# jackyko1991/vnet-tensorflow

Measured on AMD Instinct MI355X. Metric: training patches/sec (128^3x1ch fp32), higher is better.
Workload: dtype f32

## Files before the change

### include/vnet_hip.h

```cpp
#ifndef VNET_HIP_H
#define VNET_HIP_H
#include <stddef.h>
#include <stdint.h>

#ifdef __cplusplus
extern "C" {
#endif

#define VNET_OK            0
#define VNET_E_BADARG     -1
#define VNET_E_UNSUPPORTED -2
#define VNET_E_WORKSPACE  -3

#define VNET_ACT_NONE  0
#define VNET_ACT_RELU  1
#define VNET_ACT_PRELU 2
#define VNET_ACT_LRELU 3

#define VNET_PACK_FWD  0
#define VNET_PACK_BWD  1
#define VNET_PACK_UP   2

#define VNET_PACK_FWD_BF16 3
#define VNET_PACK_BWD_BF16 4
// ... 9 lines not shown
#define VNET_LOSS_SORENSEN 0
#define VNET_LOSS_JACCARD  1
#define VNET_LOSS_XENT     2
#define VNET_LOSS_WEIGHTED 16
#define VNET_LOSS_MIXED    32

const char* vnet_version(void);

double vnet_set_option(const char* name, double value);
double vnet_get_option(const char* name);

size_t vnet_packed_weight_floats(int mode, int taps, int I, int O);
int vnet_pack_weights(int mode, const float* w, float* wp, int taps, int I, int O, void* stream);
int vnet_packed_dims(int mode, int taps, int I, int O, int* CQ, int* NP);
int vnet_pack_weights_batched(const void* descs_dev, int n, void* stream);

size_t vnet_conv_ws_bytes(int ks, int kx, int stride, int up, int Cin, int Cout, int B, int Do, int Ho, int Wo);
int vnet_conv_fwd(int ks, int kx, int stride, int up, const float* x0, int C0, const float* x1, int C1, const float* wp,
    const float* bias, float* y0, int Cy0, float* y1, int Cy1, int B, int Di, int Hi, int Wi, int Do, int Ho, int Wo, void* ws,
    size_t ws_bytes, void* stream);

int vnet_conv_fwd_acc(int ks, int kx, int stride, int up, const float* x0, int C0, const float* x1, int C1, const float* wp,
    const float* bias, float* y0, int Cy0, float* y1, int Cy1, int B, int Di, int Hi, int Wi, int Do, int Ho, int Wo, void* ws,
    size_t ws_bytes, void* stream);

int vnet_conv_stats_rows(int ks, int kx, int stride, int up, int Cin, int Cy0, int Cy1, int B, int Do, int Ho, int Wo);
int vnet_conv_stats_from_reduce(int ks, int kx, int stride, int Cin, int Cout, int B, int Do, int Ho, int Wo);
int vnet_conv_fwd_stats(int ks, int kx, int stride, const float* x0, int C0, const float* x1, int C1, const float* wp,
    const float* bias, float* y, int Cout, int B, int Di, int Hi, int Wi, int Do, int Ho, int Wo, const float* res, float* stats,
    void* ws, size_t ws_bytes, void* stream);

int vnet_conv_x3_ok(int C0, int C1, int Cy0, int Cy1, int B, int D, int H, int W);
int vnet_conv_x3_stats_rows(int Cin, int Cout, int B, int D, int H, int W);
size_t vnet_conv_x3_ws_bytes(int Cin, int Cout, int B, int D, int H, int W);
int vnet_conv_fwd_x3(const float* x0, int C0, const float* x1, int C1, const void* wp, const float* bias, float* y0, int Cy0,
    float* y1, int Cy1, int B, int D, int H, int W, const float* acc, const float* res, float* stats, void* ws, size_t ws_bytes,
    void* stream);

int vnet_wgrad_x3_ok(int C0, int C1, int Cout, int B, int D, int H, int W);
size_t vnet_wgrad_x3_ws_bytes(int Cin, int Cout, int B, int D, int H, int W);
int vnet_conv_wgrad_x3(const float* x0, int C0, const float* x1, int C1, const float* dy, int Cout, float* dw, int B, int D, int H,
    int W, void* ws, size_t ws_bytes, void* stream);

size_t vnet_wgrad_bf16_ws_bytes(int Cin, int Cout, int B, int D, int H, int W);

int vnet_wgrad_defer(int on, void* stream);
int vnet_wgrad_pending(void* stream);
int vnet_wgrad_flush(void* stream);

size_t vnet_wgrad_ws_bytes(int ks, int kx, int stride, int Cin, int Cout, int B, int Do, int Ho, int Wo);
int vnet_conv_wgrad(int ks, int kx, int stride, const float* x0, int C0, const float* x1, int C1, const float* dy, int Cout,
    float* dw, int B, int Di, int Hi, int Wi, int Do, int Ho, int Wo, void* ws, size_t ws_bytes, void* stream);

int vnet_tile_im2col_x(const float* img, float* xv, int B, int D, int H, int W, void* stream);
int vnet_input_conv_fold(const float* w, const float* gamma, const float* beta, const float* mean, const float* invstd, float* wv,
    int C, int O, void* stream);
int vnet_input_conv_grads(const float* G, const float* w, const float* gamma, const float* beta, const float* mean,
    const float* invstd, float* dw, float* dgamma, float* dbeta, int C, int O, int accumulate, void* stream);

int vnet_input_conv_direct_ok(int O, int B, int D, int H, int W);
int vnet_input_conv_direct_stats_rows(int B, int D, int H, int W);
int vnet_input_conv_fold_border(const float* wv, int O, float* wbc , float* cbc , void* stream);
int vnet_input_conv_direct_fwd(const float* img, const float* wv, const float* wbc, const float* cbc, const float* bias, const float* res,
    float* y, float* stats, int O, int B, int D, int H, int W, void* stream);
int vnet_input_wgrad_direct_slabs(int B, int D, int H, int W);
int vnet_input_wgrad_direct(const float* img, const float* dy, float* G, int O, int B, int D, int H, int W, void* ws, size_t ws_bytes,
// ... 150 lines not shown
```

### vnet_tensorflow_amd/_lib.py

```python
import ctypes
import os
import subprocess

_HERE = os.path.dirname(os.path.abspath(__file__))
LIB_PATH = os.environ.get("VNET_HIP_LIB") or os.path.join(_HERE, "libvnet_hip.so")
CSRC = os.path.join(_HERE, "csrc")

_vp, _i, _i64, _f, _sz, _u64, _d = (ctypes.c_void_p, ctypes.c_int, ctypes.c_int64, ctypes.c_float,
                                    ctypes.c_size_t, ctypes.c_uint64, ctypes.c_double)

SIGNATURES = {
    "vnet_version": (ctypes.c_char_p, []),
    "vnet_set_option": (_d, [ctypes.c_char_p, _d]),
    "vnet_get_option": (_d, [ctypes.c_char_p]),
    "vnet_packed_weight_floats": (_sz, [_i, _i, _i, _i]),
    "vnet_pack_weights": (_i, [_i, _vp, _vp, _i, _i, _i, _vp]),
    "vnet_packed_dims": (_i, [_i, _i, _i, _i, ctypes.POINTER(ctypes.c_int), ctypes.POINTER(ctypes.c_int)]),
    "vnet_pack_weights_batched": (_i, [_vp, _i, _vp]),
    "vnet_conv_x3_ok": (_i, [_i] * 8),
    "vnet_conv_x3_stats_rows": (_i, [_i] * 6),
    "vnet_conv_x3_ws_bytes": (_sz, [_i] * 6),
    "vnet_conv_fwd_x3": (_i, [_vp, _i, _vp, _i, _vp, _vp, _vp, _i, _vp, _i, _i, _i, _i, _i, _vp, _vp, _vp, _vp, _sz, _vp]),
    "vnet_wgrad_x3_ok": (_i, [_i] * 7),
    "vnet_wgrad_x3_ws_bytes": (_sz, [_i] * 6),
    "vnet_conv_wgrad_x3": (_i, [_vp, _i, _vp, _i, _vp, _i, _vp, _i, _i, _i, _i, _vp, _sz, _vp]),
    "vnet_conv_ws_bytes": (_sz, [_i, _i, _i, _i, _i, _i, _i, _i, _i, _i]),
    "vnet_conv_fwd": (_i, [_i, _i, _i, _i, _vp, _i, _vp, _i, _vp, _vp, _vp, _i, _vp, _i,
                           _i, _i, _i, _i, _i, _i, _i, _vp, _sz, _vp]),
    "vnet_conv_fwd_acc": (_i, [_i, _i, _i, _i, _vp, _i, _vp, _i, _vp, _vp, _vp, _i, _vp, _i,
                               _i, _i, _i, _i, _i, _i, _i, _vp, _sz, _vp]),
    "vnet_conv_stats_rows": (_i, [_i] * 11),
    "vnet_conv_stats_from_reduce": (_i, [_i] * 9),
    "vnet_conv_fwd_stats": (_i, [_i, _i, _i, _vp, _i, _vp, _i, _vp, _vp, _vp, _i,
                                 _i, _i, _i, _i, _i, _i, _i, _vp, _vp, _vp, _sz, _vp]),
    "vnet_bn_finalize_partial": (_i, [_vp, _i, _i, _d, _f, _f, _vp, _vp, _vp, _vp, _vp]),
    "vnet_colsum_b16_ws_bytes": (_sz, [_i]),
    "vnet_colsum_b16": (_i, [_vp, _vp, _i64, _i, _vp, _sz, _vp]),
    "vnet_conv_b16_ws_bytes": (_sz, [_i] * 8),
    "vnet_conv_b16_stats_rows": (_i, [_i] * 8),
    "vnet_wgrad_bf16_ws_bytes": (_sz, [_i, _i, _i, _i, _i, _i]),
    "vnet_wgrad_defer": (_i, [_i, _vp]),
    "vnet_wgrad_pending": (_i, [_vp]),
    "vnet_wgrad_flush": (_i, [_vp]),
    "vnet_wgrad_ws_bytes": (_sz, [_i, _i, _i, _i, _i, _i, _i, _i, _i]),
    "vnet_conv_wgrad": (_i, [_i, _i, _i, _vp, _i, _vp, _i, _vp, _i, _vp,
                             _i, _i, _i, _i, _i, _i, _i, _vp, _sz, _vp]),
    "vnet_tile_im2col_x": (_i, [_vp, _vp, _i, _i, _i, _i, _vp]),
    "vnet_input_conv_fold": (_i, [_vp, _vp, _vp, _vp, _vp, _vp, _i, _i, _vp]),
    "vnet_input_conv_grads": (_i, [_vp, _vp, _vp, _vp, _vp, _vp, _vp, _vp, _vp, _i, _i, _i, _vp]),
    "vnet_input_conv_direct_ok": (_i, [_i, _i, _i, _i, _i]),
    "vnet_input_conv_direct_stats_rows": (_i, [_i, _i, _i, _i]),
    "vnet_input_conv_fold_border": (_i, [_vp, _i, _vp, _vp, _vp]),
    "vnet_input_conv_direct_fwd": (_i, [_vp, _vp, _vp, _vp, _vp, _vp, _vp, _vp, _i, _i, _i, _i, _i, _vp]),
# ... 140 lines not shown
```

### vnet_tensorflow_amd/csrc/conv_kernels.h

```cpp
#pragma once
#include "common.h"
#include <mutex>
#include <unordered_map>
#include <type_traits>
#include <vector>

namespace {

struct ConvArgs {
    const float* x0; const float* x1; int C0, C1, Cin;
    const float4* wp; const float* bias;
    float* y0; float* y1; int Cy0, Cy1, Cout;
    int B, Di, Hi, Wi, Do, Ho, Wo;
    int CQ;
    int CoutP;
    int nchunks, cps;
    int nbz, nby, nbx;
    int pad, padx;
    int vec_in, vec_out;
    float* part; size_t part_stride;
    int upO;
    int nz;
    int accum;
    const float* accsrc;
    float* stats; const float* res;
    int in4;
};

#ifdef VNET_STAMPS
static __device__ long long* g_stamps = nullptr;
#define VNET_STAMP_DECL long long ts[12]; bool stamp_on = false
#define VNET_STAMP_STEP(step) stamp_on = blockIdx.x == 88 && (step) >= 4 && (step) < 8
#define VNET_STAMP(k) do { if (stamp_on) ts[k] = __builtin_readcyclecounter(); } while (0)
#define VNET_STAMP_FLUSH(step, wave, lane, n) do { if (stamp_on && (lane) == 0 && g_stamps) { \
        for (int q_ = 0; q_ < (n); ++q_) g_stamps[(((step) - 4) * 8 + (wave)) * 12 + q_] = ts[q_]; } } while (0)
#else
#define VNET_STAMP_DECL
#define VNET_STAMP_STEP(step)
#define VNET_STAMP(k) do {} while (0)
#define VNET_STAMP_FLUSH(step, wave, lane, n) do {} while (0)
#endif

__device__ __forceinline__ float row16_sum(float v) {
    v += __builtin_bit_cast(float, __builtin_amdgcn_update_dpp(0, __builtin_bit_cast(int, v), 0xB1, 0xf, 0xf, true));
    v += __builtin_bit_cast(float, __builtin_amdgcn_update_dpp(0, __builtin_bit_cast(int, v), 0x4E, 0xf, 0xf, true));
    v += __builtin_bit_cast(float, __builtin_amdgcn_update_dpp(0, __builtin_bit_cast(int, v), 0x141, 0xf, 0xf, true));
    v += __builtin_bit_cast(float, __builtin_amdgcn_update_dpp(0, __builtin_bit_cast(int, v), 0x140, 0xf, 0xf, true));
    return v;
}
__device__ __forceinline__ float half32_sum(float v) {
    v = row16_sum(v);
    return v + __shfl_xor(v, 16, 64);
}

template <int WAVES_, int CW>
__device__ __forceinline__ void stats_row_write(const float* red, float* __restrict__ stats, size_t row, int co0, int Cout, int tid) {
    if (tid < 2 * CW) {
        float t = 0.f;
#pragma unroll
        for (int w = 0; w < WAVES_; ++w) t += red[w * 2 * CW + tid];
        const int a2 = tid / CW, c = co0 + (tid - a2 * CW);
        if (c < Cout) stats[row * 2 * Cout + (size_t)a2 * Cout + c] = t;
    }
}

__device__ __forceinline__ float bf_lo(uint32_t w) { return __uint_as_float(w << 16); }
__device__ __forceinline__ float bf_hi(uint32_t w) { return __uint_as_float(w & 0xffff0000u); }
template <bool STATS>
__device__ __forceinline__ void epilogue4_b16(const ConvArgs& a, size_t ov, int co, float (&e)[4], float* s1, float* s2) {
    unsigned short* y = (co < a.Cy0) ? reinterpret_cast<unsigned short*>(a.y0) + ov * a.Cy0 + co
                                     : reinterpret_cast<unsigned short*>(a.y1) + ov * a.Cy1 + (co - a.Cy0);
    if (a.accum) {
        const unsigned short* src = a.accsrc ? reinterpret_cast<const unsigned short*>(a.accsrc) + ov * a.Cy0 + co : y;
        const uint2 o = *reinterpret_cast<const uint2*>(src);
        e[0] += bf_lo(o.x); e[1] += bf_hi(o.x); e[2] += bf_lo(o.y); e[3] += bf_hi(o.y);
    }
    const uint2 pk = make_uint2(pk_bf16(e[0], e[1]), pk_bf16(e[2], e[3]));
    if constexpr (STATS) {
        float v[4] = {bf_lo(pk.x), bf_hi(pk.x), bf_lo(pk.y), bf_hi(pk.y)};
        if (a.res) {
            const uint2 r = *reinterpret_cast<const uint2*>(reinterpret_cast<const unsigned short*>(a.res) + ov * a.Cout + co);
            v[0] += bf_lo(r.x); v[1] += bf_hi(r.x); v[2] += bf_lo(r.y); v[3] += bf_hi(r.y);
        }
#pragma unroll
        for (int k = 0; k < 4; ++k) { s1[k] += v[k]; s2[k] += v[k] * v[k]; }
    }
    *reinterpret_cast<uint2*>(y) = pk;
}

template <bool STATS, int N>
__device__ __forceinline__ void epilogue_b16_batch(const ConvArgs& a, const size_t (&ov)[N], const int (&co)[N], const bool (&ok)[N],
                                                   float (&e)[N][4]) {
    unsigned short* y[N];
    uint2 old[N], rr[N];
#pragma unroll
// ... 520 lines not shown
        if (sg == 0 && idx < total) {
            float out[W];
#pragma unroll
            for (int j = 0; j < W; ++j) out[j] = sh[0][o * W + j] + sh[1][o * W + j] + sh[2][o * W + j] + sh[3][o * W + j];
            if (VEC) *reinterpret_cast<float4*>(dw + idx * 4) = make_float4(out[0], out[W > 1 ? 1 : 0], out[W > 2 ? 2 : 0], out[W > 3 ? 3 : 0]);
            else dw[idx] = out[0];
        }
    }
}

template <bool VEC>
__global__ void __launch_bounds__(256) wgrad_reduce_kernel(const float* __restrict__ part, int nsplit, int T3, int CinP, int CoutP,
                                                           int Cin, int Cout, float* __restrict__ dw) {
    wgrad_reduce_body<VEC>(part, nsplit, T3, CinP, CoutP, Cin, Cout, dw, blockIdx.x, gridDim.x);
}

}
namespace vnet_detail {
struct ReduceJob { const float* part; float* dw; int nsplit, T3, CinP, CoutP, Cin, Cout, vec; unsigned blk0; };
constexpr int REDUCE_BATCH = 32;
struct ReduceBatch { ReduceJob job[REDUCE_BATCH]; int n; };
struct DeferQueue { bool on = false; std::vector<ReduceJob> pending; };
struct DeferState { std::mutex mu; std::unordered_map<hipStream_t, DeferQueue> q; };
__attribute__((visibility("hidden"))) DeferState& defer_state();
struct Tuning {
    int wgrad_zs;
    int wgrad_rr;
    int conv_in4;
    double group_rounds;
    int group_debug;
    int bf16_deep;
    int bf16_deep_target;
    int bf16_c16pp;
    int x3_nb2;
    int f32_small;
};
__attribute__((visibility("hidden"))) Tuning& tuning();
}
namespace {
using vnet_detail::ReduceJob; using vnet_detail::ReduceBatch; using vnet_detail::REDUCE_BATCH;
using vnet_detail::DeferState; using vnet_detail::DeferQueue; using vnet_detail::defer_state; using vnet_detail::tuning;

__global__ void __launch_bounds__(256) wgrad_reduce_batched_kernel(ReduceBatch b) {
    int j = 0;
#pragma unroll 1
    for (int k = 1; k < b.n; ++k) if (blockIdx.x >= b.job[k].blk0) j = k;
    const ReduceJob& q = b.job[j];
    const unsigned nblk = (j + 1 < b.n ? b.job[j + 1].blk0 : gridDim.x) - q.blk0;
    if (q.vec) wgrad_reduce_body<true>(q.part, q.nsplit, q.T3, q.CinP, q.CoutP, q.Cin, q.Cout, q.dw, blockIdx.x - q.blk0, nblk);
    else wgrad_reduce_body<false>(q.part, q.nsplit, q.T3, q.CinP, q.CoutP, q.Cin, q.Cout, q.dw, blockIdx.x - q.blk0, nblk);
}


int launch_wgrad_reduce(const float* part, int nsplit, int T3, int CinP, int CoutP, int Cin, int Cout, float* dw, hipStream_t st) {
    const bool vec = (Cout % 4 == 0) && (CoutP % 4 == 0) && ((reinterpret_cast<uintptr_t>(dw) | reinterpret_cast<uintptr_t>(part)) & 15) == 0;
    {
        DeferState& ds = defer_state();
        std::lock_guard<std::mutex> lk(ds.mu);
        auto it = ds.q.find(st);
        if (it != ds.q.end() && it->second.on) {
            it->second.pending.push_back(ReduceJob{part, dw, nsplit, T3, CinP, CoutP, Cin, Cout, vec ? 1 : 0, 0u});
            return 0;
        }
    }
    const size_t total = (size_t)T3 * Cin * Cout / (vec ? 4 : 1);
    const int blocks = (int)min((size_t)4096, (total + 63) / 64);
// ... 1638 lines not shown
```

### vnet_tensorflow_amd/csrc/conv_mfma.hip

```cpp
#include "conv_kernels.h"
#include <string.h>

namespace vnet_detail {
DeferState& defer_state() { static DeferState s; return s; }
static Tuning tuning_from_env() {
    auto geti = [](const char* n, int d) { const char* e = getenv(n); return e ? atoi(e) : d; };
    Tuning t{};
    t.wgrad_zs = geti("VNET_WGRAD_ZS", 2); t.wgrad_rr = geti("VNET_WGRAD_RR", 1); t.conv_in4 = geti("VNET_CONV_IN4", 1);
    const char* g = getenv("VNET_WGRAD_GROUP_ROUNDS");
    t.group_rounds = g ? atof(g) : 2.0;
    t.group_debug = getenv("VNET_WGRAD_GROUP_DEBUG") ? 1 : 0;
    t.bf16_deep = geti("VNET_BF16_DEEP", 1); t.bf16_deep_target = geti("VNET_BF16_DEEP_TARGET", 256);
    t.f32_small = geti("VNET_F32_SMALL", 2); t.x3_nb2 = geti("VNET_X3_NB2", 1); t.bf16_c16pp = geti("VNET_BF16_C16PP", 1);
    return t;
}
Tuning& tuning() { static Tuning t = tuning_from_env(); return t; }
}

namespace {
double* option_slot(const char* name, int** ip) {
    vnet_detail::Tuning& t = vnet_detail::tuning();
    *ip = nullptr;
    if (!name) return nullptr;
    if (!strcmp(name, "WGRAD_ZS")) *ip = &t.wgrad_zs;
    else if (!strcmp(name, "WGRAD_RR")) *ip = &t.wgrad_rr;
    else if (!strcmp(name, "CONV_IN4")) *ip = &t.conv_in4;
    else if (!strcmp(name, "WGRAD_GROUP_DEBUG")) *ip = &t.group_debug;
    else if (!strcmp(name, "BF16_DEEP")) *ip = &t.bf16_deep;
    else if (!strcmp(name, "BF16_DEEP_TARGET")) *ip = &t.bf16_deep_target;
    else if (!strcmp(name, "F32_SMALL")) *ip = &t.f32_small;
    else if (!strcmp(name, "X3_NB2")) *ip = &t.x3_nb2;
    else if (!strcmp(name, "BF16_C16PP")) *ip = &t.bf16_c16pp;
    else if (!strcmp(name, "WGRAD_GROUP_ROUNDS")) return &t.group_rounds;
    return nullptr;
}
}

extern "C" {

double vnet_set_option(const char* name, double value) {
    int* ip; double* dp = option_slot(name, &ip);
    if (ip) { const double prev = *ip; *ip = (int)value; return prev; }
    if (dp) { const double prev = *dp; *dp = value; return prev; }
    return __builtin_nan("");
}
double vnet_get_option(const char* name) {
    int* ip; double* dp = option_slot(name, &ip);
    return ip ? (double)*ip : (dp ? *dp : __builtin_nan(""));
}

const char* vnet_version(void) { return "vnet_hip 0.2 (gfx950; fp32 MFMA 16x16x4, bf16 MFMA 32x32x16 / 16x16x32)"; }

size_t vnet_packed_weight_floats(int mode, int taps, int I, int O) {
    if (mode == VNET_PACK_FWD_X3 || mode == VNET_PACK_BWD_X3) {
        int nchunk, ncob; x3_packed_dims(mode == VNET_PACK_BWD_X3, I, O, &nchunk, &ncob);
        return (size_t)nchunk * X3_NPAIR * ncob * 3 * 256;
    }
    if (mode == VNET_PACK_FWD_BF16 || mode == VNET_PACK_BWD_BF16) {
        int nchunk, ncob; packed_dims_bf16(mode, I, O, &nchunk, &ncob);
        return (size_t)nchunk * taps * ncob * 512 / 2;
    }
    int Tp, CQ, NP; packed_dims(mode & ~VNET_PACK_ROUND_BF16, taps, I, O, &Tp, &CQ, &NP);
    return (size_t)Tp * CQ * NP * 4;
}

// ... 267 lines not shown
```

### vnet_tensorflow_amd/csrc/conv_x3.h

```cpp
#pragma once
#include "conv_kernels.h"

namespace {

constexpr int X3_TZ = 2, X3_TY = 8, X3_TX = 16;
constexpr int X3_IZ = X3_TZ + 4, X3_IY = X3_TY + 4, X3_IX = X3_TX + 4;
constexpr int X3_NV = X3_IZ * X3_IY * X3_IX;

template <bool W8>
struct X3G {
    static constexpr int TZ = W8 ? 4 : 2;
    static constexpr int IZ = TZ + 4, IY = X3_IY, IX = W8 ? 12 : X3_IX;
    static constexpr int ROWB = IX * 16;
    static constexpr int ZB = IY * ROWB + (W8 ? 64 : 0);
    static constexpr int PLANEB = IZ * ZB;
    static constexpr int PIECEB = 2 * PLANEB;
    static constexpr int TILEB = 3 * PIECEB;
    static constexpr int LDS = TILEB + 2 * 8 * 32 * 4;
    static constexpr int SPER = W8 ? 8 : 12;
};
static_assert(X3G<false>::PLANEB == X3_NV * 16 && X3G<false>::PLANEB % 256 == 0 && X3G<true>::PLANEB % 256 == 0, "tile planes");
static_assert((2 * X3G<true>::ZB) % 256 == 128, "lanes 8..15 of the narrow brick: the other half of the 256-byte bank row");
constexpr int X3_LDS = X3G<false>::LDS;

template <int K, int N, typename F>
__device__ __forceinline__ void x3_for_impl(F&& f) {
    if constexpr (K < N) { f(std::integral_constant<int, K>{}); x3_for_impl<K + 1, N>(f); }
}
template <int N, typename F>
__device__ __forceinline__ void x3_for(F&& f) { x3_for_impl<0, N>(f); }

typedef const __attribute__((address_space(1))) u32x4* x3_gw_t;
template <int NP>
__device__ __forceinline__ void x3_load_a(bf16x8 (&A)[NP][3], const u32x4* __restrict__ wbase, unsigned u0, unsigned ustride, int lane) {
    x3_for<NP * 3>([&](auto I) {
        constexpr int p = decltype(I)::value / 3, s = decltype(I)::value % 3;
        A[p][s] = __builtin_bit_cast(bf16x8, *(x3_gw_t)(wbase + (u0 + (unsigned)p * ustride + (unsigned)s * 64u) + lane));
    });
}
__device__ __forceinline__ void x3_load_a1(bf16x8 (&A)[3], const u32x4* __restrict__ wbase, unsigned u0, int lane) {
    x3_for<3>([&](auto I) {
        constexpr int s = decltype(I)::value;
        A[s] = __builtin_bit_cast(bf16x8, *(x3_gw_t)(wbase + (u0 + (unsigned)s * 64u) + lane));
    });
}

template <typename G>
__device__ __forceinline__ void x3_read_b(bf16x8 (&B)[3], const unsigned char* p) {
    B[0] = *reinterpret_cast<const bf16x8*>(p);
    B[1] = *reinterpret_cast<const bf16x8*>(p + G::PIECEB);
    B[2] = *reinterpret_cast<const bf16x8*>(p + 2 * G::PIECEB);
// ... 25 lines not shown
__device__ __forceinline__ void x3_yrows_pairs(f32x4 (&acc)[8], const unsigned char* by, const bf16x8 (&A)[NA][3]) {
    bf16x8 Bn[3];
    x3_read_b<G>(Bn, by);
    x3_for<10>([&](auto KI) {
        constexpr int k = decltype(KI)::value;
        bf16x8 B[3] = {Bn[0], Bn[1], Bn[2]};
        if constexpr (k + 1 < 10) x3_read_b<G>(Bn, by + (k + 1) * G::ROWB);
        __builtin_amdgcn_sched_barrier(0);
        x3_for<6>([&](auto TI) {
            constexpr int t = decltype(TI)::value;
            if constexpr (k < 8) acc[k] = __builtin_amdgcn_mfma_f32_16x16x32_bf16(A[A0][X3_PROD_A(t)], B[X3_PROD_B(t)], acc[k], 0, 0, 0);
            if constexpr (k >= 2) acc[k - 2] = __builtin_amdgcn_mfma_f32_16x16x32_bf16(A[A0 + 1][X3_PROD_A(t)], B[X3_PROD_B(t)], acc[k - 2], 0, 0, 0);
        });
        __builtin_amdgcn_sched_barrier(0);
    });
}
template <typename G, int A0, int NA>
__device__ __forceinline__ void x3_yrows_single(f32x4 (&acc)[8], const unsigned char* b0, const bf16x8 (&A)[NA][3]) {
    bf16x8 Bn[3];
    x3_read_b<G>(Bn, b0 + 4 * G::ROWB);
    x3_for<8>([&](auto MI) {
        constexpr int m = decltype(MI)::value;
        bf16x8 B[3] = {Bn[0], Bn[1], Bn[2]};
        if constexpr (m + 1 < 8) x3_read_b<G>(Bn, b0 + (m + 5) * G::ROWB);
        __builtin_amdgcn_sched_barrier(0);
        x3_for<6>([&](auto TI) {
            constexpr int t = decltype(TI)::value;
            acc[m] = __builtin_amdgcn_mfma_f32_16x16x32_bf16(A[A0][X3_PROD_A(t)], B[X3_PROD_B(t)], acc[m], 0, 0, 0);
        });
        __builtin_amdgcn_sched_barrier(0);
    });
}

template <bool STATS, int NB, bool W8 = false>
__global__ void __launch_bounds__(512) __attribute__((amdgpu_waves_per_eu(2, 2))) conv5_x3_kernel(ConvArgs a) {
    constexpr int NT = 512;
    using G = X3G<W8>;
    using XT = XTile<X3_IZ, X3_IY, X3_IX, NT>;
    static_assert(XT::PER * XT::RPI == XT::ROWS && XT::PER == X3G<false>::SPER, "every staging pass covers whole tile rows");
    extern __shared__ __attribute__((aligned(16))) unsigned char smem[];
    unsigned char* tile = smem;
    float* red = reinterpret_cast<float*>(smem);
    float* sred = reinterpret_cast<float*>(smem + G::TILEB);
    const int tid = threadIdx.x;
    const int lane = tid & 63, wave = __builtin_amdgcn_readfirstlane(tid >> 6);
    const int j = lane & 15, g = lane >> 4, half = g & 1, hi = g >> 1;
    const int grp = wave >> 2, kw = wave & 3;

    const int base0 = W8 ? half * G::PLANEB + (grp + 2 * (j >> 3)) * G::ZB + (j & 7) * 16
                         : half * G::PLANEB + ((grp * G::IY) * G::IX + j) * 16;
    const unsigned char* bZ = tile + base0 + hi * G::ZB;
    const unsigned char* bY = tile + base0 + hi * G::ROWB + 4 * G::ZB;
    const unsigned char* b0 = tile + base0 + 4 * G::ZB;
    const unsigned char* bX = b0 + hi * 16;

    const int ncob = a.CoutP >> 4, ncobg = ncob / NB;
    const int nbrick = a.B * a.nbz * a.nby * a.nbx;
    const int nks = a.nz;
    const int nitems = nbrick * ncobg * nks;
    const int G8 = gridDim.x >> 3;
    const int per_xcd = (nitems + 7) >> 3;
    const int xcd = blockIdx.x & 7, slot = blockIdx.x >> 3;
    const int i_lo = xcd * per_xcd, i_hi = min(nitems, i_lo + per_xcd);
    if (i_lo + slot >= i_hi) return;
    const int nmine = (i_hi - i_lo - slot + G8 - 1) / G8;
    const int nch = a.cps;
    const int nsteps = nmine * nch;
    const unsigned astride = (unsigned)ncob * 3u * 64u;
    const u32x4* wbase = reinterpret_cast<const u32x4*>(a.wp);

    auto item_coords = [&](int it, int& b, int& bz, int& by, int& bx, int& cob) {
        int item = (i_lo + slot + it * G8) / nks;
        cob = (item % ncobg) * NB; item /= ncobg;
        bx = item % a.nbx; item /= a.nbx;
        by = item % a.nby; item /= a.nby;
        bz = item % a.nbz; b = item / a.nbz;
    };
    typedef const __attribute__((address_space(1))) f32x4* gf4_t;
    f32x4 pv[G::SPER];
    const int stid = W8 ? (tid < 384 ? tid : tid - 128) : (tid < XT::RPI * XT::COLS ? tid : tid - XT::COLS);
    constexpr int SCOLS = W8 ? 32 : XT::COLS;
    const int sr0 = stid / SCOLS, scol = stid - sr0 * SCOLS;
    const int six = scol >> 2, scq = scol & 3;
    auto tile_issue = [&](int step) {
        const int it = step / nch, ch = ((i_lo + slot + it * G8) % nks) * nch + (step - it * nch);
        int b, bz, by, bx, cob;
        item_coords(it, b, bz, by, bx, cob);
        const int c0 = ch * 16;
        const bool first = c0 < a.C0;
        const int cs = first ? a.C0 : a.C1;
        const float* src = (first ? a.x0 + c0 : a.x1 + (c0 - a.C0)) + (size_t)b * a.Di * a.Hi * a.Wi * cs;
        if constexpr (W8) {
            const int gz0 = bz * G::TZ - 2, gy = by * X3_TY - 2 + sr0;
            const bool yok = (unsigned)gy < (unsigned)a.Hi;
            const int rs = a.Wi * cs;
            const int off0 = (gy * a.Wi + six) * cs + scq * 4;
// ... 151 lines not shown
                const int oy = by * X3_TY + 2 * kw + t;
                if (oz < a.Do && oy < a.Ho && ox < a.Wo && co < a.Cout) {
                    const size_t ov = ((size_t)(b * a.Do + oz) * a.Ho + oy) * a.Wo + ox;
                    if (a.part) {
                        *reinterpret_cast<f32x4*>(a.part + (size_t)ks * a.part_stride + ov * a.CoutP + co) = o[t];
                        return;
                    }
                    float e[4] = {o[t][0] + bias4[0], o[t][1] + bias4[1], o[t][2] + bias4[2], o[t][3] + bias4[3]};
                    if constexpr (STATS) {
                        float4 rr = make_float4(0.f, 0.f, 0.f, 0.f);
                        if (a.res) rr = *reinterpret_cast<const float4*>(a.res + ov * a.Cout + co);
                        const float vv[4] = {e[0] + rr.x, e[1] + rr.y, e[2] + rr.z, e[3] + rr.w};
                        s1[0] += vv[0]; s1[1] += vv[1]; s1[2] += vv[2]; s1[3] += vv[3];
                        s2[0] += vv[0] * vv[0]; s2[1] += vv[1] * vv[1]; s2[2] += vv[2] * vv[2]; s2[3] += vv[3] * vv[3];
                    }
                    float* p = (co < a.Cy0) ? a.y0 + ov * a.Cy0 + co : a.y1 + ov * a.Cy1 + (co - a.Cy0);
                    if (a.accum) {
                        const float4 old = *reinterpret_cast<const float4*>(a.accsrc ? a.accsrc + ov * a.Cy0 + co : p);
                        e[0] += old.x; e[1] += old.y; e[2] += old.z; e[3] += old.w;
                    }
                    *reinterpret_cast<float4*>(p) = make_float4(e[0], e[1], e[2], e[3]);
                }
            });
            if constexpr (STATS) {
                x3_for<4>([&](auto KI) {
                    constexpr int k = decltype(KI)::value;
                    s1[k] = row16_sum(s1[k]); s2[k] = row16_sum(s2[k]);
                    if (j == 0) { sred[(nb * 8 + wave) * 32 + 4 * g + k] = s1[k]; sred[(nb * 8 + wave) * 32 + 16 + 4 * g + k] = s2[k]; }
                });
            }
            });
            __syncthreads();
            if constexpr (STATS) {
                int brick = (i_lo + slot + it * G8) / (ncobg * nks);
                x3_for<NB>([&](auto NBI) {
                    constexpr int nb = decltype(NBI)::value;
                    stats_row_write<8, 16>(sred + nb * 8 * 32, a.stats, (size_t)brick, (cob + nb) * 16, a.Cout, tid);
                });
            }
        }
        VNET_STAMP(6);
        if (last) zero_halo();
        if (more) tile_commit(((last ? 0 : lc + 1) & 1) ? 0x80000000u : 0u);
        VNET_STAMP(7);
        __syncthreads();
        VNET_STAMP(8);
        VNET_STAMP_FLUSH(step, wave, lane, 9);
    }
}

template <bool W8>
struct XWG {
    static constexpr int TZ = W8 ? 4 : 2;
    static constexpr int IZ = TZ + 4, IX = W8 ? 12 : X3_IX;
    static constexpr int XROW = IX * 32, XPLANE = X3_IY * XROW;
    static constexpr int XPB = IZ * XPLANE;
    static constexpr int DPB = 2 * X3_TY * 16 * 32;
    static constexpr int LDS = 3 * XPB + 3 * DPB;
    static constexpr int XHALF = W8 ? 2 * XPLANE : 8 * 32;
    static constexpr int XPER = W8 ? 8 : 12;
};
static_assert(XWG<false>::XROW % 256 == 128 && XWG<true>::XROW % 256 == 128, "row pairs of a k-step on disjoint banks");
constexpr int XW_LDS = XWG<false>::LDS;

__device__ __forceinline__ void xw_frag(bf16x8 (&F)[3], const unsigned char* lo, const unsigned char* hi, int pieceb) {
    typedef s16x4 __attribute__((address_space(3))) * lp;
#pragma unroll
    for (int s = 0; s < 3; ++s) {
        const s16x4 a = __builtin_amdgcn_ds_read_tr16_b64_v4i16((lp)(lo + s * pieceb));
        const s16x4 b = __builtin_amdgcn_ds_read_tr16_b64_v4i16((lp)(hi + s * pieceb));
        const s16x8 v = {a[0], a[1], a[2], a[3], b[0], b[1], b[2], b[3]};
        F[s] = __builtin_bit_cast(bf16x8, v);
    }
}

__device__ __forceinline__ void xw_mfma6(f32x4& acc, const bf16x8 (&A)[3], const bf16x8 (&B)[3]) {
#pragma unroll
    for (int k = 0; k < 6; ++k) acc = __builtin_amdgcn_mfma_f32_16x16x32_bf16(A[X3_PROD_A(k)], B[X3_PROD_B(k)], acc, 0, 0, 0);
}

// ... 241 lines not shown
```

### vnet_tensorflow_amd/csrc/conv_x3.hip

```cpp
#include "conv_x3.h"

namespace {

int x3_grid() { return device_cus() / 8 * 8; }

}

extern "C" {

int vnet_conv_x3_ok(int C0, int C1, int Cy0, int Cy1, int B, int D, int H, int W) {
    return x3_conv_ok(C0, C1, Cy0, Cy1, B, D, H, W) ? 1 : 0;
}

int vnet_conv_x3_stats_rows(int Cin, int Cout, int B, int D, int H, int W) {
    if (Cin <= 0 || Cout <= 0 || B <= 0 || D <= 0 || H <= 0 || W <= 0) return 0;
    const X3Plan p = x3_plan_conv(Cin, 0, Cout, 0, B, D, H, W);
    if (p.nks > 1) {
        if (Cout > 256 || 256 % Cout) return 0;
        const size_t total = (size_t)B * D * H * W * Cout;
        return (int)min((size_t)2048, (total + 255) / 256);
    }
    return x3_conv_bricks(B, D, H, W);
}

size_t vnet_conv_x3_ws_bytes(int Cin, int Cout, int B, int D, int H, int W) {
    if (Cin <= 0 || Cout <= 0 || (Cin & 15) || (Cout & 15) || B <= 0 || D <= 0 || H <= 0 || W <= 0) return 0;
    const X3Plan p = x3_plan_conv(Cin, 0, Cout, 0, B, D, H, W);
    return p.nks > 1 ? (size_t)p.nks * B * D * H * W * Cout * sizeof(float) : 0;
}

int vnet_conv_fwd_x3(const float* x0, int C0, const float* x1, int C1, const void* wp, const float* bias,
                     float* y0, int Cy0, float* y1, int Cy1, int B, int D, int H, int W,
                     const float* acc, const float* res, float* stats, void* ws, size_t ws_bytes, void* stream) {
    if (!x0 || !wp || !y0 || C0 <= 0 || Cy0 <= 0 || B <= 0 || D <= 0 || H <= 0 || W <= 0) return VNET_E_BADARG;
    if ((C1 > 0 && !x1) || (Cy1 > 0 && !y1) || C1 < 0 || Cy1 < 0) return VNET_E_BADARG;
    if ((C0 & 15) || (C1 & 15) || (Cy0 & 15) || (Cy1 & 15)) return VNET_E_UNSUPPORTED;
    if ((stats || res) && Cy1 > 0) return VNET_E_BADARG;
    if (acc && acc != y0 && Cy1 > 0) return VNET_E_BADARG;
    if ((long long)D * H * W * (C0 > C1 ? C0 : C1) >= (1ll << 31)) return VNET_E_UNSUPPORTED;
    ConvArgs a{};
    a.x0 = x0; a.x1 = x1; a.C0 = C0; a.C1 = C1; a.Cin = C0 + C1;
    a.wp = reinterpret_cast<const float4*>(wp); a.bias = bias;
    a.y0 = y0; a.y1 = y1; a.Cy0 = Cy0; a.Cy1 = Cy1; a.Cout = Cy0 + Cy1;
    a.B = B; a.Di = D; a.Hi = H; a.Wi = W; a.Do = D; a.Ho = H; a.Wo = W;
    a.nchunks = a.Cin / 16; a.CQ = a.nchunks * 4; a.CoutP = a.Cout;
    a.nbz = x3_conv_nbz(D, W); a.nby = ceil_div(H, X3_TY); a.nbx = ceil_div(W, X3_TX);
    a.pad = 2; a.padx = 2; a.vec_in = 1; a.vec_out = 1;
    a.accum = acc ? 1 : 0; a.accsrc = (acc && acc != y0) ? acc : nullptr;
    a.res = res; a.stats = stats;
    const X3Plan p = x3_plan_conv(a.Cin, 0, a.Cout, 0, B, D, H, W);
    a.nz = p.nks; a.cps = p.cps ? p.cps : a.nchunks;
    const size_t nvox = (size_t)B * D * H * W;
    if (p.nks > 1) {
        const size_t need = (size_t)p.nks * nvox * a.Cout * sizeof(float);
        if (!ws || ws_bytes < need) return VNET_E_WORKSPACE;
        if (stats && (a.Cout > 256 || 256 % a.Cout)) return VNET_E_UNSUPPORTED;
        a.part = reinterpret_cast<float*>(ws); a.part_stride = nvox * a.Cout;
    }
    hipStream_t st = (hipStream_t)stream;
    const int grid = x3_grid();
    const bool w8 = W == 8;
    const bool nb2 = !w8 && (a.Cout % 32 == 0) && p.items * p.nks >= 2 * (long)grid && tuning().x3_nb2 != 0;
    const int e = with_bool(stats && p.nks == 1, [&](auto S) {
        return w8 ? launch<conv5_x3_kernel<S, 1, true>>(dim3(grid), dim3(512), X3G<true>::LDS, st, a)
                  : with_int<2, 1>(nb2 ? 2 : 1, [&](auto NB) {
                        return launch<conv5_x3_kernel<S, NB, false>>(dim3(grid), dim3(512), X3G<false>::LDS, st, a);
                    });
    });
    if (e || p.nks <= 1) return e;
    const size_t total = nvox * a.Cout;
    const int blocks = (int)min((size_t)2048, (total + 255) / 256);
    return launch<splitk_reduce_kernel>(dim3(blocks), dim3(256), 0, st, a.part, a.part_stride, p.nks, bias,
                                        y0, y1, Cy0, Cy1, a.CoutP, nvox, a.accum, a.res, a.stats, a.accsrc);
}

int vnet_wgrad_x3_ok(int C0, int C1, int Cout, int B, int D, int H, int W) {
    return x3_wgrad_ok(C0, C1, Cout, B, D, H, W) ? 1 : 0;
}

size_t vnet_wgrad_x3_ws_bytes(int Cin, int Cout, int B, int D, int H, int W) {
    if (Cin <= 0 || Cout <= 0 || (Cin & 15) || (Cout & 15) || B <= 0 || D <= 0 || H <= 0 || W <= 0) return 0;
    const X3WgradPlan p = x3_plan_wgrad(Cin, Cout, B, D, H, W);
    return (size_t)p.nsplit * 125 * Cin * Cout * sizeof(float);
}

int vnet_conv_wgrad_x3(const float* x0, int C0, const float* x1, int C1, const float* dy, int Cout, float* dw,
                       int B, int D, int H, int W, void* ws, size_t ws_bytes, void* stream) {
    if (!x0 || !dy || !dw || C0 <= 0 || Cout <= 0 || B <= 0 || C1 < 0 || (C1 > 0 && !x1)) return VNET_E_BADARG;
    if (D <= 0 || H <= 0 || W <= 0) return VNET_E_BADARG;
    if ((C0 & 15) || (C1 & 15) || (Cout & 15)) return VNET_E_UNSUPPORTED;
    if ((long long)D * H * W * (C0 > C1 ? C0 : C1) >= (1ll << 31)) return VNET_E_UNSUPPORTED;
    hipStream_t st = (hipStream_t)stream;
    WgradArgs a{};
    a.x0 = x0; a.x1 = x1; a.C0 = C0; a.C1 = C1; a.Cin = C0 + C1; a.dy = dy; a.Cout = Cout;
    a.B = B; a.Di = D; a.Hi = H; a.Wi = W; a.Do = D; a.Ho = H; a.Wo = W;
    a.CinP = a.Cin; a.CoutP = Cout; a.pad = 2; a.padx = 2; a.vec_in = 1; a.vec_dy = 1;
    const X3WgradPlan p = x3_plan_wgrad(a.Cin, Cout, B, D, H, W);
    a.ncob = Cout / 16; a.nbz = p.nbz; a.nby = p.nby; a.nbx = p.nbx; a.nbrick = p.nbrick; a.nsplit = p.nsplit;
    const size_t need = (size_t)p.nsplit * 125 * a.Cin * Cout * sizeof(float);
    const bool direct = p.nsplit == 1;
// ... 13 lines not shown
```

### vnet_tensorflow_amd/ops.py

```python
import collections
import contextlib
import ctypes
import math
import os as _os
import weakref

import torch

from . import _lib
from ._lib import VnetHipError, check

BN_EPS = 1e-3
BN_MOMENTUM = 0.99

ACT = {None: 0, "none": 0, "relu": 1, "prelu": 2, "lrelu": 3}
PACK_FWD, PACK_BWD, PACK_UP, PACK_FWD_BF16, PACK_BWD_BF16, PACK_BOTH_BF16, PACK_BOTH = 0, 1, 2, 3, 4, 5, 6
PACK_FWD_X3, PACK_BWD_X3, PACK_BOTH_X3 = 7, 8, 9

class OpsContext(object):
    def __init__(self):
        self.compute = {"dtype": "fp32", "store16": False, "name": "fp32", "split3": False}
        self.pg = {"on": False, "streams": {}, "used": set(), "keep": []}
        self.pack_epoch = [0]
        self.pack_reg = {"entries": [], "descs": None, "device": None}
# ... 904 lines not shown
                                              _ptr(gs.view), _ptr(bs.view), C, O, int(accumulate), _stream()), "vnet_input_conv_grads")
                _grad_ret(dw, sw)
                if not accumulate:
                    _grad_ret(gs.view, gs)
                    _grad_ret(bs.view, bs)
            gpar._vnet_deferred = deferred

            def flush(gpar=gpar):
                th = getattr(gpar, "_vnet_deferred", None)
                if th is not None:
                    del gpar._vnet_deferred
                    th(0)
            torch.autograd.Variable._execution_engine.queue_callback(flush)
            return None, None, None, None, None, None, _grad_ret(db, sb), None, None, None
        dgamma = torch.empty(C, dtype=torch.float32, device=dev)
        dbeta = torch.empty(C, dtype=torch.float32, device=dev)
        check(L.vnet_input_conv_grads(_ptr(G), _ptr(w), _ptr(gamma), _ptr(beta), _ptr(mean), _ptr(invstd), _ptr(dw),
                                      _ptr(dgamma), _ptr(dbeta), C, O, 0, _stream()), "vnet_input_conv_grads")
        return None, dgamma, dbeta, None, None, _grad_ret(dw, sw), _grad_ret(db, sb), None, None, None


class _EpilogueStats(object):
    __slots__ = ("partial", "rows", "residual")

    def __init__(self, partial, rows, residual):
        self.partial, self.rows, self.residual = partial, rows, residual


def _with_epilogue_stats(fn, args, r, O, bn_stats, bn_residual, device):
    if not (bn_stats and _FUSE["bn_stats"] and _SYNC_BN is None and r.stats_rows > 0):
        return fn.apply(*args)
    stats = torch.empty((r.stats_rows, 2 * O), dtype=torch.float32, device=device)
    y = fn.apply(*args, stats, bn_residual)
    y._vnet_stats = _EpilogueStats(stats, r.stats_rows, bn_residual)
    return y


def input_conv(img, gamma, beta, mean, invstd, w, b, bn_stats=False, bn_residual=None):
    if _meta(img):
        return torch.empty(img.shape[:-1] + (w.shape[-1],), device="meta")
    _need_gpu(img, "input_conv")
    B, D, H, W, _ = img.shape
    r = route(IN_FWD, 5, 1, 0, False, False, 1, 0, w.shape[-1], B, (D, H, W), (D, H, W))
    return _with_epilogue_stats(_InputConvFn, (img, gamma, beta, mean, invstd, w, b, r), r, w.shape[-1], bn_stats, bn_residual, img.device)


def conv(x0, w, b, ks, stride=1, x1=None, bn_stats=False, bn_residual=None):
    if x0.dim() != 5:
        raise NotImplementedError("only the 3-D (NDHWC) path is built; 2-D is out of scope (SURVEY section 2 row 11)")
    if _meta(x0):
        B, D, H, W, _ = x0.shape
        return torch.empty((B, _same_out(D, stride), _same_out(H, stride), _same_out(W, stride), w.shape[-1]), device="meta")
    _need_gpu(x0, "conv", allow16=True)
    fused = bn_stats and _FUSE["bn_stats"] and _SYNC_BN is None
    r = _conv_route(FWD, x0, x1, w, ks, stride, False, tuple(_same_out(int(v), stride) for v in x0.shape[1:4]),
                    res=fused and bn_residual is not None)
    return _with_epilogue_stats(_ConvFn, (x0, x1, w, b, r), r, w.shape[-1], bn_stats, bn_residual, x0.device)


def conv_transpose2(x, w, b, out_spatial):
    if x.dim() != 5:
        raise NotImplementedError("only the 3-D (NDHWC) path is built")
    if _meta(x):
        return torch.empty((x.shape[0],) + tuple(out_spatial) + (w.shape[-2],), device="meta")
    _need_gpu(x, "conv_transpose2", allow16=True)
    return _ConvFn.apply(x, None, w, b, _conv_route(FWD, x, None, w, 2, 2, True, out_spatial))

# ... 579 lines not shown
```

Measured before the change: 66.70.

## Accumulate BN stats per workgroup in LDS for x3 conv kernel

Instead of writing one BN-statistics row per brick to global memory, each persistent workgroup of the x3 conv kernel accumulates its partial sums in shared memory and writes a single row at the end. The downstream finalize reduces only grid-count rows (a live-rows query is exposed to Python), which cuts global stats traffic and reduction work. Rows beyond the grid are zeroed so the existing buffer size stays valid. This adds LDS usage per block, which could affect occupancy, plus extra zero-fill writes.

```diff
diff --git a/include/vnet_hip.h b/include/vnet_hip.h
--- a/include/vnet_hip.h
+++ b/include/vnet_hip.h
@@ -65,6 +65,7 @@
 
 int vnet_conv_x3_ok(int C0, int C1, int Cy0, int Cy1, int B, int D, int H, int W);
 int vnet_conv_x3_stats_rows(int Cin, int Cout, int B, int D, int H, int W);
+int vnet_conv_x3_stats_rows_live(int Cin, int Cout, int B, int D, int H, int W);
 size_t vnet_conv_x3_ws_bytes(int Cin, int Cout, int B, int D, int H, int W);
 int vnet_conv_fwd_x3(const float* x0, int C0, const float* x1, int C1, const void* wp, const float* bias, float* y0, int Cy0,
     float* y1, int Cy1, int B, int D, int H, int W, const float* acc, const float* res, float* stats, void* ws, size_t ws_bytes,
diff --git a/vnet_tensorflow_amd/_lib.py b/vnet_tensorflow_amd/_lib.py
--- a/vnet_tensorflow_amd/_lib.py
+++ b/vnet_tensorflow_amd/_lib.py
@@ -19,6 +19,7 @@
     "vnet_pack_weights_batched": (_i, [_vp, _i, _vp]),
     "vnet_conv_x3_ok": (_i, [_i] * 8),
     "vnet_conv_x3_stats_rows": (_i, [_i] * 6),
+    "vnet_conv_x3_stats_rows_live": (_i, [_i] * 6),
     "vnet_conv_x3_ws_bytes": (_sz, [_i] * 6),
     "vnet_conv_fwd_x3": (_i, [_vp, _i, _vp, _i, _vp, _vp, _vp, _i, _vp, _i, _i, _i, _i, _i, _vp, _vp, _vp, _vp, _sz, _vp]),
     "vnet_wgrad_x3_ok": (_i, [_i] * 7),
diff --git a/vnet_tensorflow_amd/csrc/conv_kernels.h b/vnet_tensorflow_amd/csrc/conv_kernels.h
--- a/vnet_tensorflow_amd/csrc/conv_kernels.h
+++ b/vnet_tensorflow_amd/csrc/conv_kernels.h
@@ -24,6 +24,7 @@
     int accum;
     const float* accsrc;
     float* stats; const float* res;
+    int stats_wg;
     int in4;
 };
 
@@ -61,6 +62,16 @@
         for (int w = 0; w < WAVES_; ++w) t += red[w * 2 * CW + tid];
         const int a2 = tid / CW, c = co0 + (tid - a2 * CW);
         if (c < Cout) stats[row * 2 * Cout + (size_t)a2 * Cout + c] = t;
+    }
+}
+template <int WAVES_, int CW>
+__device__ __forceinline__ void stats_row_add(const float* red, float* wsum, int co0, int Cout, int tid) {
+    if (tid < 2 * CW) {
+        float t = 0.f;
+#pragma unroll
+        for (int w = 0; w < WAVES_; ++w) t += red[w * 2 * CW + tid];
+        const int a2 = tid / CW, c = co0 + (tid - a2 * CW);
+        if (c < Cout) wsum[a2 * Cout + c] += t;
     }
 }
 
@@ -647,6 +658,7 @@
     int bf16_deep;
     int bf16_deep_target;
     int bf16_c16pp;
+    int x3_stats_wg;
     int x3_nb2;
     int f32_small;
 };
diff --git a/vnet_tensorflow_amd/csrc/conv_mfma.hip b/vnet_tensorflow_amd/csrc/conv_mfma.hip
--- a/vnet_tensorflow_amd/csrc/conv_mfma.hip
+++ b/vnet_tensorflow_amd/csrc/conv_mfma.hip
@@ -12,6 +12,7 @@
     t.group_debug = getenv("VNET_WGRAD_GROUP_DEBUG") ? 1 : 0;
     t.bf16_deep = geti("VNET_BF16_DEEP", 1); t.bf16_deep_target = geti("VNET_BF16_DEEP_TARGET", 256);
     t.f32_small = geti("VNET_F32_SMALL", 2); t.x3_nb2 = geti("VNET_X3_NB2", 1); t.bf16_c16pp = geti("VNET_BF16_C16PP", 1);
+    t.x3_stats_wg = geti("VNET_X3_STATS_WG", 1);
     return t;
 }
 Tuning& tuning() { static Tuning t = tuning_from_env(); return t; }
@@ -31,6 +32,7 @@
     else if (!strcmp(name, "F32_SMALL")) *ip = &t.f32_small;
     else if (!strcmp(name, "X3_NB2")) *ip = &t.x3_nb2;
     else if (!strcmp(name, "BF16_C16PP")) *ip = &t.bf16_c16pp;
+    else if (!strcmp(name, "X3_STATS_WG")) *ip = &t.x3_stats_wg;
     else if (!strcmp(name, "WGRAD_GROUP_ROUNDS")) return &t.group_rounds;
     return nullptr;
 }
diff --git a/vnet_tensorflow_amd/csrc/conv_x3.h b/vnet_tensorflow_amd/csrc/conv_x3.h
--- a/vnet_tensorflow_amd/csrc/conv_x3.h
+++ b/vnet_tensorflow_amd/csrc/conv_x3.h
@@ -16,7 +16,8 @@
     static constexpr int PLANEB = IZ * ZB;
     static constexpr int PIECEB = 2 * PLANEB;
     static constexpr int TILEB = 3 * PIECEB;
-    static constexpr int LDS = TILEB + 2 * 8 * 32 * 4;
+    static constexpr int SREDB = 2 * 8 * 32 * 4;
+    static constexpr int LDS = TILEB + SREDB + 2 * 256 * 4;
     static constexpr int SPER = W8 ? 8 : 12;
 };
 static_assert(X3G<false>::PLANEB == X3_NV * 16 && X3G<false>::PLANEB % 256 == 0 && X3G<true>::PLANEB % 256 == 0, "tile planes");
@@ -108,7 +109,7 @@
     });
 }
 
-template <bool STATS, int NB, bool W8 = false>
+template <bool STATS, int NB, bool W8 = false, bool WG = false>
 __global__ void __launch_bounds__(512) __attribute__((amdgpu_waves_per_eu(2, 2))) conv5_x3_kernel(ConvArgs a) {
     constexpr int NT = 512;
     using G = X3G<W8>;
@@ -138,6 +139,19 @@
     const int per_xcd = (nitems + 7) >> 3;
     const int xcd = blockIdx.x & 7, slot = blockIdx.x >> 3;
     const int i_lo = xcd * per_xcd, i_hi = min(nitems, i_lo + per_xcd);
+    float* wsum = reinterpret_cast<float*>(smem + G::TILEB + G::SREDB);
+    [[maybe_unused]] auto zero_rows_behind = [&]() {
+        for (int row = blockIdx.x + gridDim.x; row < nbrick; row += gridDim.x)
+            for (int i = tid; i < 2 * a.Cout; i += NT) a.stats[(size_t)row * 2 * a.Cout + i] = 0.f;
+    };
+    if constexpr (STATS && WG) {
+        if (i_lo + slot >= i_hi) {
+            for (int i = tid; i < 2 * a.Cout; i += NT) a.stats[(size_t)blockIdx.x * 2 * a.Cout + i] = 0.f;
+            zero_rows_behind();
+        } else {
+            for (int i = tid; i < 2 * a.Cout; i += NT) wsum[i] = 0.f;
+        }
+    }
     if (i_lo + slot >= i_hi) return;
     const int nmine = (i_hi - i_lo - slot + G8 - 1) / G8;
     const int nch = a.cps;
@@ -355,10 +369,11 @@
             });
             __syncthreads();
             if constexpr (STATS) {
-                int brick = (i_lo + slot + it * G8) / (ncobg * nks);
+                [[maybe_unused]] int brick = (i_lo + slot + it * G8) / (ncobg * nks);
                 x3_for<NB>([&](auto NBI) {
                     constexpr int nb = decltype(NBI)::value;
-                    stats_row_write<8, 16>(sred + nb * 8 * 32, a.stats, (size_t)brick, (cob + nb) * 16, a.Cout, tid);
+                    if constexpr (WG) stats_row_add<8, 16>(sred + nb * 8 * 32, wsum, (cob + nb) * 16, a.Cout, tid);
+                    else stats_row_write<8, 16>(sred + nb * 8 * 32, a.stats, (size_t)brick, (cob + nb) * 16, a.Cout, tid);
                 });
             }
         }
@@ -369,6 +384,10 @@
         __syncthreads();
         VNET_STAMP(8);
         VNET_STAMP_FLUSH(step, wave, lane, 9);
+    }
+    if constexpr (STATS && WG) {
+        for (int i = tid; i < 2 * a.Cout; i += NT) a.stats[(size_t)blockIdx.x * 2 * a.Cout + i] = wsum[i];
+        zero_rows_behind();
     }
 }
 
diff --git a/vnet_tensorflow_amd/csrc/conv_x3.hip b/vnet_tensorflow_amd/csrc/conv_x3.hip
--- a/vnet_tensorflow_amd/csrc/conv_x3.hip
+++ b/vnet_tensorflow_amd/csrc/conv_x3.hip
@@ -3,6 +3,10 @@
 namespace {
 
 int x3_grid() { return device_cus() / 8 * 8; }
+
+bool x3_stats_per_wg(int Cout, int B, int D, int H, int W) {
+    return tuning().x3_stats_wg != 0 && Cout <= 256 && x3_conv_bricks(B, D, H, W) > x3_grid();
+}
 
 }
 
@@ -21,6 +25,13 @@
         return (int)min((size_t)2048, (total + 255) / 256);
     }
     return x3_conv_bricks(B, D, H, W);
+}
+
+int vnet_conv_x3_stats_rows_live(int Cin, int Cout, int B, int D, int H, int W) {
+    const int rows = vnet_conv_x3_stats_rows(Cin, Cout, B, D, H, W);
+    if (rows <= 0) return rows;
+    const X3Plan p = x3_plan_conv(Cin, 0, Cout, 0, B, D, H, W);
+    return p.nks == 1 && x3_stats_per_wg(Cout, B, D, H, W) ? x3_grid() : rows;
 }
 
 size_t vnet_conv_x3_ws_bytes(int Cin, int Cout, int B, int D, int H, int W) {
@@ -50,6 +61,7 @@
     a.res = res; a.stats = stats;
     const X3Plan p = x3_plan_conv(a.Cin, 0, a.Cout, 0, B, D, H, W);
     a.nz = p.nks; a.cps = p.cps ? p.cps : a.nchunks;
+    a.stats_wg = stats && p.nks == 1 && x3_stats_per_wg(a.Cout, B, D, H, W);
     const size_t nvox = (size_t)B * D * H * W;
     if (p.nks > 1) {
         const size_t need = (size_t)p.nks * nvox * a.Cout * sizeof(float);
@@ -62,10 +74,13 @@
     const bool w8 = W == 8;
     const bool nb2 = !w8 && (a.Cout % 32 == 0) && p.items * p.nks >= 2 * (long)grid && tuning().x3_nb2 != 0;
     const int e = with_bool(stats && p.nks == 1, [&](auto S) {
-        return w8 ? launch<conv5_x3_kernel<S, 1, true>>(dim3(grid), dim3(512), X3G<true>::LDS, st, a)
-                  : with_int<2, 1>(nb2 ? 2 : 1, [&](auto NB) {
-                        return launch<conv5_x3_kernel<S, NB, false>>(dim3(grid), dim3(512), X3G<false>::LDS, st, a);
-                    });
+        return with_bool(a.stats_wg != 0, [&](auto WG) {
+            constexpr bool wg = S && WG;
+            return w8 ? launch<conv5_x3_kernel<S, 1, true, wg>>(dim3(grid), dim3(512), X3G<true>::LDS, st, a)
+                      : with_int<2, 1>(nb2 ? 2 : 1, [&](auto NB) {
+                            return launch<conv5_x3_kernel<S, NB, false, wg>>(dim3(grid), dim3(512), X3G<false>::LDS, st, a);
+                        });
+        });
     });
     if (e || p.nks <= 1) return e;
     const size_t total = nvox * a.Cout;
diff --git a/vnet_tensorflow_amd/ops.py b/vnet_tensorflow_amd/ops.py
--- a/vnet_tensorflow_amd/ops.py
+++ b/vnet_tensorflow_amd/ops.py
@@ -960,7 +960,10 @@
         return fn.apply(*args)
     stats = torch.empty((r.stats_rows, 2 * O), dtype=torch.float32, device=device)
     y = fn.apply(*args, stats, bn_residual)
-    y._vnet_stats = _EpilogueStats(stats, r.stats_rows, bn_residual)
+    rows = r.stats_rows
+    if r.family == "conv-x3":
+        rows = _lib.lib().vnet_conv_x3_stats_rows_live(r.cin, O, int(y.shape[0]), *r.dout)
+    y._vnet_stats = _EpilogueStats(stats, rows, bn_residual)
     return y
 
 
```

After: 66.75, median of 2. No clear change (+0.1%).
